# liruihui/Dis-PU

Hardware: AMD Instinct MI355X
Metric: upsampled points/sec (256->1024, 4x) (higher is better)
Workload: dtype f32; 1 GPU; BASELINE configs[1]: 32 patches x 256 points per GPU, generator forward 256->1024 (4x), fp32; patches_per_gpu=32, global_patches=32, weights=xavier-uniform seed 1234, zero bias, parallelism=patch-sharded x1

## Files before the change

### dis-pu_amd/_lib.py

```python
import ctypes as C
import os

_HERE = os.path.dirname(os.path.abspath(__file__))
LIB_PATH = os.path.join(_HERE, "lib", "libdispu_hip.so")

ABI_VERSION = 5
ARITH_PLAIN = 0
ARITH_CONTRACT = 1
ARITH_PINNED_EXP = 2
MESH_BRUTE_FORCE = 8
MESH_TILE = 64

_vp, _i, _sz, _l = C.c_void_p, C.c_int, C.c_size_t, C.c_long

SIGNATURES = {
    "dispu_version": (_i, []),
    "dispu_error_string": (C.c_char_p, [_i]),
    "dispu_event_record": (_i, [_vp, _vp]),
    "dispu_stream_wait_event": (_i, [_vp, _vp]),
    "dispu_memset_async": (_i, [_vp, _i, _sz, _vp]),
    "dispu_fps_scratch_bytes": (_sz, [_i, _i, _i]),
    "dispu_fps": (_i, [_i, _i, _i, _vp, _vp, _vp, _i, _vp]),
    "dispu_fps_ws": (_i, [_i, _i, _i, _vp, _vp, _sz, _vp, _i, _vp]),
    "dispu_fps_segments_scratch_bytes": (_sz, [_i, _vp, _vp]),
# ... 39 lines not shown
    "dispu_sa_fused": (_i, [_i, _i, _i, _i, _i, _vp, _vp, _vp, _vp, _i, _vp, _vp, _vp, _vp, _vp, _vp, _vp]),
    "dispu_edge_conv_fused": (_i, [_i, _i, _i, _i, _vp, _l, _vp, _i, _i, _vp, _vp, _vp, _vp, _vp, _i, _vp, _vp]),
    "dispu_group_center": (_i, [_l, _i, _i, _vp, _vp, _vp]),
    "dispu_pool_nsample": (_i, [_l, _i, _i, _i, _vp, _vp, _vp, _vp]),
    "dispu_idw_weights": (_i, [_l, _vp, _vp, _vp]),
    "dispu_l2_normalize_rows": (_i, [_l, _i, _vp, _vp, _vp]),
    "dispu_scale_add": (_i, [_l, _vp, C.c_float, _vp, _vp, _vp]),
    "dispu_edge_feature": (_i, [_l, _i, _i, _i, _vp, _l, _vp, _i, _i, _vp, _l, _vp]),
    "dispu_row_mean_max": (_i, [_i, _i, _vp, _vp, _vp, _vp]),
    "dispu_repulsion": (_i, [_l, _i, _i, _i, C.c_float, _vp, _vp, _vp, _vp]),
    "dispu_linear_small_k": (_i, [_l, _i, _i, _vp, _l, _vp, _vp, _i, _vp, _l, _vp]),
    "dispu_linear_small_n": (_i, [_l, _i, _i, _vp, _l, _vp, _vp, _i, _vp, _l, _vp, _l, _vp]),
    "dispu_edge_dense_conv": (_i, [_i, _i, _i, _vp, _l, _vp, _i, _i, _vp, _vp, _vp, _vp, _vp, _vp, _vp, _l, _vp]),
    "dispu_stem_block": (_i, [_i, _i, _i, _vp, _l, _i, _i, _vp, _vp, _vp, _vp, _vp, _vp, _vp, _l, _vp, _vp, _vp, _i, _vp, _l, _vp, _vp, _vp, _vp,
                              _l, _vp]),
    "dispu_edge_dense_conv_valu": (_i, [_i, _i, _i, _vp, _l, _vp, _i, _i, _vp, _vp, _vp, _vp, _vp, _vp, _vp, _l, _vp]),
    "dispu_dup_grid": (_i, [_i, _i, _i, _i, _vp, _l, _vp, _vp, _vp, _vp, _l, _vp]),
    "dispu_ps_prep": (_i, [_l, _i, _vp, _vp, _vp, _vp, _l, _vp, _l, _vp]),
    "dispu_ps_gather_sub_relu": (_i, [_l, _i, _i, _i, _vp, _vp, _l, _vp, _l, _vp, _l, _vp]),
    "dispu_ps_skip_max": (_i, [_l, _i, _i, _i, _vp, _vp, _vp, _l, _vp, _l, _vp]),
    "dispu_ps_weight_net": (_i, [_l, _i, _i, _i, _vp, _vp, _vp, _vp, _vp, _vp, _vp, _vp]),
    "dispu_ps_point_matmul": (_i, [_l, _i, _i, _i, _vp, _l, _vp, _vp, _l, _vp]),
    "dispu_ps_local": (_i, [_l, _i, _i, _i, _vp, _vp, _vp, _l, _vp, _vp, _vp, _vp, _vp, _vp, _vp, _vp, _vp]),
    "dispu_knn_patch": (_i, [_i, _i, _i, _i, _vp, _vp, _vp, _vp]),
    "dispu_normalize_patches": (_i, [_i, _i, _vp, _vp, _vp, _vp, _vp]),
    "dispu_denormalize_patches": (_i, [_i, _i, _vp, _vp, _vp, _vp, _vp]),
    "dispu_knn_patch_segments": (_i, [_i, _vp, _vp, _vp, _vp, _i, _vp, _vp, _vp, _vp]),
    "dispu_normalize_segments": (_i, [_i, _vp, _vp, _vp, _vp, _vp, _vp, _vp]),
    "dispu_attention": (_i, [_i, _i, _i, _i, _vp, _l, _vp, _l, _vp, _l, C.c_float, _vp, _l, _vp]),
    "dispu_attention_fwd_lse": (_i, [_i, _i, _i, _i, _vp, _l, _vp, _l, _vp, _l, C.c_float, _vp, _l, _vp, _vp]),
    "dispu_attention_bwd": (_i, [_i, _i, _i, _i, _vp, _l, _vp, _l, _vp, _l, C.c_float, _vp, _l, _vp, _vp, _l, _vp, _l, _vp, _l, _vp, _l,
                                 _vp, _vp]),
    "dispu_attention_project": (_i, [_i, _i, _i, _i, _vp, _l, _vp, _l, _vp, _l, C.c_float, _vp, _vp, _i, _vp, _l, _vp]),
    "dispu_softmax_rows": (_i, [_l, _i, C.c_float, _vp, _l, _vp]),
    "dispu_linear_tn_bf16_stream_scratch_floats": (_l, [_i, _i, _i]),
    "dispu_linear_tn_bf16_stream": (_i, [_i, _i, _i, _vp, _l, _vp, _l, _i, _vp, _l, _i, _vp, _vp, _l, _vp]),
    "dispu_bf16_pack": (_i, [_i, _i, _vp, _l, _i, _vp, _vp]),
    "dispu_linear_bf16_stream": (_i, [_i, _i, _i, _vp, _l, _i, _vp, _l, _vp, _i, _vp, _l, _i, _i, _l, _vp]),
    "dispu_linear_bf16": (_i, [_i, _i, _i, _i, _vp, _l, _l, _vp, _l, _l, _i, _vp, _i, _vp, _l, _l, _vp, _l, _l, _vp, _l, _l, _vp]),
    "dispu_linear_tn_bf16_scratch_floats": (_l, [_i, _i, _i, _i]),
    "dispu_linear_tn_bf16": (_i, [_i, _i, _i, _i, _vp, _l, _l, _vp, _l, _l, _vp, _l, _l, _i, _vp, _vp, _l, _vp]),
    "dispu_bf16x3_split_weights": (_i, [_i, _i, _vp, _l, _vp, _vp]),
    "dispu_linear_bf16x3": (_i, [_i, _i, _i, _vp, _l, _vp, _vp, _i, _vp, _l, _vp, _l, _vp, _l, _vp]),
    "dispu_debug_x3_kernel": (None, [_i]),
    "dispu_linear_tn_scratch_floats": (_l, [_i, _i, _i, _i]),
    "dispu_linear_tn": (_i, [_i, _i, _i, _i, _vp, _l, _l, _vp, _l, _l, _vp, _l, _l, _i, _vp, _vp, _l, _vp]),
    "dispu_ps_local_grad": (_i, [_l, _i] + [_vp] * 3 + [_l] + [_vp] * 14),
    "dispu_tn_defer": (_i, [_vp]),
    "dispu_tn_reduce_grouped": (_i, [_i, _vp, _vp, _vp]),
    "dispu_act_bias_grad_scratch_floats": (_l, [_l, _i]),
    "dispu_act_bias_grad": (_i, [_l, _i, _vp, _l, _vp, _l, _i, _vp, _l, _vp, _i, _vp, _l, _vp]),
    "dispu_max_k": (_i, [_l, _i, _i, _vp, _l, _vp, _l, _vp]),
    "dispu_max_k_grad": (_i, [_l, _i, _i, _vp, _l, _vp, _l, _vp, _l, _vp, _l, _i, _vp]),
    "dispu_max_k_grad_tail": (_i, [_l, _i, _i, _i, _vp, _l, _vp, _l, _vp, _l, _vp, _l, _vp]),
    "dispu_edge_feature_grad": (_i, [_l, _i, _i, _i, _vp, _l, _vp, _i, _i, _vp, _l, _vp]),
    "dispu_dup_sum_grad": (_i, [_i, _i, _i, _i, _vp, _l, _vp, _l, _vp]),
    "dispu_ps_group": (_i, [_l, _i, _i, _i, _vp, _vp, _vp, _l, _vp, _l, _vp]),
    "dispu_ps_group_grad": (_i, [_l, _i, _i, _i, _vp, _vp, _l, _vp, _vp, _l, _vp]),
    "dispu_ps_point_matmul_grad": (_i, [_l, _i, _i, _i, _vp, _l, _vp, _vp, _l, _vp, _l, _vp, _vp]),
    "dispu_softmax_rows_grad": (_i, [_l, _i, C.c_float, _vp, _l, _vp, _l, _vp]),
    "dispu_bn_scratch_bytes": (_l, [_l, _i]),
    "dispu_bn_train": (_i, [_l, _i, _vp, _l, _vp, _vp, C.c_float, C.c_float, _i, _vp, _l, _vp, _vp, _vp, _vp, _l, _vp]),
    "dispu_bn_train_grad": (_i, [_l, _i, _vp, _l, _vp, _l, _vp, _l, _vp, _vp, _i, _vp, _l, _vp, _vp, _vp, _vp, _l, _vp]),
    "dispu_sigmoid_offset": (_i, [_l, _vp, _vp, _vp, _vp]),
    "dispu_sigmoid_offset_grad": (_i, [_l, _vp, _vp, _vp, _vp, _vp]),
    "dispu_repulsion_grad": (_i, [_l, _i, _i, C.c_float, C.c_float, _vp, _vp, _vp, _vp]),
# ... 175 lines not shown
```

### dis-pu_amd/csrc/attention.hip

```cpp
#include "common.h"

namespace dispu {

typedef float f32x16 __attribute__((ext_vector_type(16)));

constexpr int FA_D = 64, FA_TK = 32, FA_LDK = FA_D + 1;
constexpr int FA_STAGE = FA_TK * FA_LDK + FA_TK * FA_D;

constexpr int FA_BPN = 256;
#ifdef FA_STAMPS
__device__ unsigned long long fa_stamps[16];
#endif

template <bool BP>
__global__ __launch_bounds__(512) void flash_attention_kernel(int m, int nk, const float* __restrict__ Q, long ldq,
                                                               const float* __restrict__ K, long ldk,
                                                               const float* __restrict__ V, long ldv, float scale,
                                                               float* __restrict__ O, long ldo,
                                                               const float* __restrict__ Wbp, const float* __restrict__ bbp) {
    extern __shared__ __attribute__((aligned(16))) float lds[];
    const int lane = threadIdx.x & 63, wave = threadIdx.x >> 6;
    int cloud = blockIdx.y, qblk = blockIdx.x;
    if ((gridDim.y & 7u) == 0) {
        const unsigned lin = blockIdx.x + gridDim.x * blockIdx.y, slot = lin >> 3;
        cloud = (int)((lin & 7u) * (gridDim.y >> 3) + slot / gridDim.x);
        qblk = (int)(slot % gridDim.x);
    }
    const float* __restrict__ kb = K + (size_t)cloud * nk * ldk;
    const float* __restrict__ vb = V + (size_t)cloud * nk * ldv;
    const int ntile = nk / FA_TK;

    if (wave >= 4) {
        const int tid = threadIdx.x - 256;
        float4 pk[2], pv[2];
        auto load_tile = [&](int k0) {
#pragma unroll
            for (int it = 0; it < 2; ++it) {
                const int e = tid + it * 256, key = e >> 4, c4 = e & 15;
                pk[it] = *reinterpret_cast<const float4*>(kb + (size_t)(k0 + key) * ldk + c4 * 4);
                pv[it] = *reinterpret_cast<const float4*>(vb + (size_t)(k0 + key) * ldv + c4 * 4);
            }
        };
        auto store_tile = [&](int stage) {
            float* Kt = lds + stage * FA_STAGE;
            float* Vt = Kt + FA_TK * FA_LDK;
#pragma unroll
            for (int it = 0; it < 2; ++it) {
                const int e = tid + it * 256, key = e >> 4, c4 = e & 15;
                Kt[key * FA_LDK + c4 * 4 + 0] = pk[it].x;
                Kt[key * FA_LDK + c4 * 4 + 1] = pk[it].y;
                Kt[key * FA_LDK + c4 * 4 + 2] = pk[it].z;
                Kt[key * FA_LDK + c4 * 4 + 3] = pk[it].w;
                *reinterpret_cast<float4*>(&Vt[key * FA_D + c4 * 4]) = pv[it];
            }
        };
        load_tile(0);
        if constexpr (BP) {
            float* Wl = lds + 2 * FA_STAGE;
#pragma unroll
            for (int h = 0; h < 4; ++h) {
                float4 w[4];
#pragma unroll
                for (int u = 0; u < 4; ++u) w[u] = *reinterpret_cast<const float4*>(Wbp + (size_t)(tid + (h * 4 + u) * 256) * 4);
#pragma unroll
                for (int u = 0; u < 4; ++u) *reinterpret_cast<float4*>(Wl + (size_t)(tid + (h * 4 + u) * 256) * 4) = w[u];
            }
        }
        store_tile(0);
        if (ntile > 1) load_tile(FA_TK);
        __syncthreads();
        for (int t = 0; t < ntile; ++t) {
            if (t + 1 < ntile) {
                store_tile((t + 1) & 1);
                if (t + 2 < ntile) load_tile((t + 2) * FA_TK);
            }
            __syncthreads();
        }
        return;
    }

    const int qrow = qblk * 128 + wave * 32 + (lane & 31);
    const int kh = lane >> 5, li = lane & 31;
    const bool qok = qrow < m;
    const float* __restrict__ qp = Q + ((size_t)cloud * m + (qok ? qrow : 0)) * ldq;

    const float scale2 = scale * 1.4426950408889634f;
    float qf[32];
#pragma unroll
    for (int s4 = 0; s4 < 16; ++s4) {
        const float4 v = *reinterpret_cast<const float4*>(qp + s4 * 4);
        qf[2 * s4] = (kh ? v.y : v.x) * scale2;
        qf[2 * s4 + 1] = (kh ? v.w : v.z) * scale2;
    }

    f32x16 oacc[2];
#pragma unroll
    for (int c = 0; c < 2; ++c)
#pragma unroll
        for (int r = 0; r < 16; ++r) oacc[c][r] = 0.f;
    float mrun = -__builtin_inff(), lsum = 0.f;

    __syncthreads();
#ifdef FA_STAMPS
    unsigned long long fa_s = 0, fa_sm = 0, fa_pv = 0, fa_bar = 0;
#define FA_T(v) __builtin_amdgcn_sched_barrier(0); const unsigned long long v = __builtin_readcyclecounter(); __builtin_amdgcn_sched_barrier(0)
#else
#define FA_T(v)
#endif
    for (int t = 0; t < ntile; ++t) {
        FA_T(c0);
        const float* Kt = lds + (t & 1) * FA_STAGE;
        const float* Vt = Kt + FA_TK * FA_LDK;
        f32x16 sacc;
#pragma unroll
        for (int r = 0; r < 16; ++r) sacc[r] = 0.f;
#pragma unroll
        for (int s = 0; s < 32; ++s) sacc = __builtin_amdgcn_mfma_f32_32x32x2f32(Kt[li * FA_LDK + 2 * s + kh], qf[s], sacc, 0, 0, 0);
        FA_T(c1);
        float mx = fmaxf(fmaxf(sacc[0], sacc[1]), sacc[2]);
#pragma unroll
        for (int r = 3; r < 15; r += 2) mx = fmaxf(fmaxf(mx, sacc[r]), sacc[r + 1]);
        mx = fmaxf(mx, sacc[15]);
        mx = fmaxf(mx, __shfl_xor(mx, 32, 64));
        const float mnew = fmaxf(mrun, mx);
        const float alpha = __builtin_amdgcn_exp2f(mrun - mnew);
        float rs = 0.f;
#pragma unroll
        for (int r = 0; r < 16; ++r) { sacc[r] = __builtin_amdgcn_exp2f(sacc[r] - mnew); rs += sacc[r]; }
        lsum = lsum * alpha + rs;
        mrun = mnew;
        if (__any(alpha != 1.0f)) {
#pragma unroll
            for (int c = 0; c < 2; ++c)
#pragma unroll
                for (int r = 0; r < 16; ++r) oacc[c][r] = oacc[c][r] * alpha;
        }
        FA_T(c2);
#pragma unroll
        for (int r = 0; r < 16; ++r) {
            const int key = (r & 3) + 8 * (r >> 2) + 4 * kh;
#pragma unroll
            for (int c = 0; c < 2; ++c)
                oacc[c] = __builtin_amdgcn_mfma_f32_32x32x2f32(Vt[key * FA_D + c * 32 + li], sacc[r], oacc[c], 0, 0, 0);
        }
        FA_T(c3);
        __syncthreads();
#ifdef FA_STAMPS
        { FA_T(c4); fa_s += c1 - c0; fa_sm += c2 - c1; fa_pv += c3 - c2; fa_bar += c4 - c3; }
#endif
    }
#ifdef FA_STAMPS
    if (blockIdx.x == 3 && blockIdx.y == 1 && lane == 0) {
        fa_stamps[wave * 4 + 0] = fa_s; fa_stamps[wave * 4 + 1] = fa_sm; fa_stamps[wave * 4 + 2] = fa_pv; fa_stamps[wave * 4 + 3] = fa_bar;
    }
#endif
    const float ltot = lsum + __shfl_xor(lsum, 32, 64);
    const float inv = 1.0f / ltot;
    float* __restrict__ op = O + ((size_t)cloud * m + (qok ? qrow : 0)) * ldo;
    if constexpr (!BP) {
        if (qok) {
#pragma unroll
            for (int c = 0; c < 2; ++c)
#pragma unroll
                for (int r = 0; r < 16; ++r) op[c * 32 + (r & 3) + 8 * (r >> 2) + 4 * kh] = oacc[c][r] * inv;
        }
    } else {
        const float* Wl = lds + 2 * FA_STAGE;
#pragma unroll
        for (int c = 0; c < 2; ++c)
#pragma unroll
            for (int r = 0; r < 16; ++r) oacc[c][r] = oacc[c][r] * inv;
#pragma unroll 1
        for (int ot = 0; ot < FA_BPN / 32; ot += 2) {
            f32x16 y0, y1;
#pragma unroll
            for (int r = 0; r < 16; ++r) { y0[r] = 0.f; y1[r] = 0.f; }
#pragma unroll
            for (int c = 0; c < 2; ++c)
#pragma unroll
                for (int r = 0; r < 16; ++r) {
                    const int d = c * 32 + (r & 3) + 8 * (r >> 2) + 4 * kh;
                    y0 = __builtin_amdgcn_mfma_f32_32x32x2f32(Wl[d * FA_BPN + ot * 32 + li], oacc[c][r], y0, 0, 0, 0);
                    y1 = __builtin_amdgcn_mfma_f32_32x32x2f32(Wl[d * FA_BPN + ot * 32 + 32 + li], oacc[c][r], y1, 0, 0, 0);
                }
            if (qok) {
#pragma unroll
                for (int g = 0; g < 4; ++g) {
                    const int o0 = ot * 32 + 8 * g + 4 * kh;
                    const float4 b0 = *reinterpret_cast<const float4*>(bbp + o0), b1 = *reinterpret_cast<const float4*>(bbp + o0 + 32);
                    float4 v0, v1;
                    v0.x = fmaxf(y0[4 * g + 0] + b0.x, 0.f); v0.y = fmaxf(y0[4 * g + 1] + b0.y, 0.f);
                    v0.z = fmaxf(y0[4 * g + 2] + b0.z, 0.f); v0.w = fmaxf(y0[4 * g + 3] + b0.w, 0.f);
                    v1.x = fmaxf(y1[4 * g + 0] + b1.x, 0.f); v1.y = fmaxf(y1[4 * g + 1] + b1.y, 0.f);
                    v1.z = fmaxf(y1[4 * g + 2] + b1.z, 0.f); v1.w = fmaxf(y1[4 * g + 3] + b1.w, 0.f);
                    *reinterpret_cast<float4*>(op + o0) = v0;
                    *reinterpret_cast<float4*>(op + o0 + 32) = v1;
                }
            }
        }
    }
}

}

using namespace dispu;

DISPU_EXPORT int dispu_attention(int b, int m, int nk, int d, const float* Q, long ldq, const float* K, long ldk, const float* V,
                                 long ldv, float scale, float* O, long ldo, void* stream) {
    if (b < 0 || m <= 0 || nk <= 0 || d != 64 || (nk % 32) != 0 || (ldq & 3) || (ldk & 3) || (ldv & 3) ||
        ((((uintptr_t)Q) | ((uintptr_t)K) | ((uintptr_t)V)) & 15))
        return (int)hipErrorInvalidValue;
    if (b == 0) return 0;
    hipLaunchKernelGGL((flash_attention_kernel<false>), dim3((m + 127) / 128, b), dim3(512), 2 * FA_STAGE * sizeof(float),
                       (hipStream_t)stream, m, nk, Q, ldq, K, ldk, V, ldv, scale, O, ldo, (const float*)nullptr, (const float*)nullptr);
    return (int)hipGetLastError();
}

DISPU_EXPORT int dispu_attention_project(int b, int m, int nk, int d, const float* Q, long ldq, const float* K, long ldk,
                                         const float* V, long ldv, float scale, const float* W, const float* bias, int n_out,
                                         float* Y, long ldy, void* stream) {
    if (b < 0 || m <= 0 || nk <= 0 || d != 64 || n_out != FA_BPN || (nk % 32) != 0 || (ldq & 3) || (ldk & 3) || (ldv & 3) ||
        (ldy & 3) || !W || !bias ||
        ((((uintptr_t)Q) | ((uintptr_t)K) | ((uintptr_t)V) | ((uintptr_t)W) | ((uintptr_t)bias) | ((uintptr_t)Y)) & 15))
        return (int)hipErrorInvalidValue;
    if (b == 0) return 0;
    constexpr size_t bytes = (size_t)(2 * FA_STAGE + FA_D * FA_BPN) * sizeof(float);
    static DevOnce attr;      
    if (attr.needed()) {
        DISPU_TRY(hipFuncSetAttribute(reinterpret_cast<const void*>(flash_attention_kernel<true>),
                                      hipFuncAttributeMaxDynamicSharedMemorySize, (int)bytes));
        attr.done();
    }
    hipLaunchKernelGGL((flash_attention_kernel<true>), dim3((m + 127) / 128, b), dim3(512), bytes, (hipStream_t)stream, m, nk, Q, ldq,
                       K, ldk, V, ldv, scale, Y, ldy, W, bias);
    return (int)hipGetLastError();
}
```

### dis-pu_amd/generator.py

```python
import contextlib
import math

import numpy as np
import torch

from . import _lib

K_NEIGH = 16
GROWTH = 24
DENSE_BLOCKS = 4
BN_EPS = 1e-3


def gen_grid(up_ratio):
    sq = int(math.sqrt(up_ratio)) + 1
    for i in range(sq, 0, -1):
        if up_ratio % i == 0:
            num_x, num_y = i, up_ratio // i
            break
    gx = np.linspace(-0.2, 0.2, num_x, dtype=np.float32)
    gy = np.linspace(-0.2, 0.2, num_y, dtype=np.float32)
    x, y = np.meshgrid(gx, gy)
    return np.stack([x, y], -1).reshape(-1, 2).astype(np.float32)


class _Opts(object):
    patch_num_point = 256
    up_ratio = 4


class Generator(object):

    MAX_POINTS = 2048 * 256

    def __init__(self, opts=None, is_training=False, name="Generator", params=None, device=None):
        self.opts = opts if opts is not None else _Opts()
        self.is_training = is_training
        self.name = name
        self.num_point = int(self.opts.patch_num_point)
        self.up_ratio = int(self.opts.up_ratio)
        if self.up_ratio != 4:
            raise NotImplementedError("the shipped generator graph is built for up_ratio 4 (DisPU/configs.py)")
        self.out_num_point = self.num_point * self.up_ratio
        self.device = torch.device(device if device is not None else "cuda:0")
        if self.device.type == "cuda" and self.device.index is None:
            self.device = torch.device("cuda", torch.cuda.current_device())
        self.P = {}
        self._ws = {}
        self.profile = None
        self.fused_local = True
        self.fused_attention = True
        self.fused_project = True
        self.split_bf16 = False
        self._planes = {}
        self.split_up3 = True
        self.branches = True
        self._aux = None
        self.fused_residual = True
        self.fused_heads = True
        self.keep_intermediates = False
        self.chain_inputs = True
        self.fused_stem = True
        self.return_views = False
        self.fine_out = None
        self._trainer = None
        if params is not None:
            self.load_params(params)

    def load_params(self, params):
        dev = self.device
        if self.is_training:
            from .train import Trainer, TrainOpts
            topts = TrainOpts()
            for k in dir(self.opts):
                if not k.startswith("_"):
                    setattr(topts, k, getattr(self.opts, k))
            self._trainer = Trainer(opts=topts, params=params, device=dev)
            self.P = self._trainer.P
            return
        self.P = {k: torch.from_numpy(np.ascontiguousarray(v, np.float32)).to(dev) for k, v in params.items()}
        self._planes = {}
        bn = "refine/PointShuffle/weight_net/wconv0/bn/"
        g, b = params[bn + "gamma"].astype(np.float64), params[bn + "beta"].astype(np.float64)
        mu, var = params[bn + "moving_mean"].astype(np.float64), params[bn + "moving_variance"].astype(np.float64)
        scale = g / np.sqrt(var + BN_EPS)
        self.bn_scale = torch.from_numpy(scale.astype(np.float32)).to(dev)
        self.bn_shift = torch.from_numpy((b - mu * scale).astype(np.float32)).to(dev)
        self.grid = torch.from_numpy(gen_grid(self.up_ratio)).to(dev)
        w1 = self.P["generator/upshuffle_0/conv1/weights"]
        self.w_up_feat = w1[:480].contiguous()
        self.w_up_grid = w1[480:482].contiguous()
        w0 = self.P["refine/PointShuffle/conv0/weights"]
        self.w_c0_feat = w0[6:134].contiguous()
        nlp = "refine/PointShuffle/PointShuffle/"
        self.w_up3 = torch.cat([self.P[nlp + "conv_kv/weights"], self.P[nlp + "conv_query/weights"], self.w_c0_feat], dim=1).contiguous()
        self.b_up3 = torch.cat([self.P[nlp + "conv_kv/biases"], self.P[nlp + "conv_query/biases"],
                                torch.zeros(128, dtype=torch.float32, device=dev)]).contiguous()
        wsk = self.P["refine/PointShuffle/skip/weights"]
        self.w_skip_pad = torch.cat([wsk, torch.zeros((10, wsk.shape[1]), dtype=torch.float32, device=dev)], dim=0).contiguous()

    def _w(self, scope):
        return self.P[scope + "/weights"], self.P[scope + "/biases"]

    def _workspace(self, B, N):
        key = (B, N)
        ws = self._ws.get(key)
        if ws is not None:
            return ws
        dev, f32, i32 = self.device, torch.float32, torch.int32
        M = N * self.up_ratio
        rn, rm, k = B * N, B * M, K_NEIGH

        def E(*shape, dtype=f32):
            return torch.empty(shape, dtype=dtype, device=dev)

        ws = dict(
            feat=E(rn, 480), prep=E(rn, 48), prep_b=E(rn, 48), kidx=E(rn, k + 1, dtype=i32), h256=E(rn, 256),
            up256=E(rm, 256), up128=E(rm, 128), c256=E(rm, 256), c64=E(rm, 64), coarse=E(B, M, 3),
            psidx=E(rm, k, dtype=i32), up3=E(rm, 320), att=E(rm, 64), nl=E(rm, 256),
            skipin=torch.zeros((rm, 144), dtype=f32, device=dev), skip=E(rm, 256), am=E(rm, 128),
            fp=E(rm, 2048), aft=E(rm, 256), agg=E(rm, 256),
            f256=E(rm, 256), f64=E(rm, 64), fine=E(B, M, 3))
        ws["kv"], ws["q"], ws["gm"] = ws["up3"][:, 0:128], ws["up3"][:, 128:192], ws["up3"][:, 192:320]
        self._ws[key] = ws
        return ws

    def _pair_buffers(self, B, N):
        key = ("pair", B, N)
        if key not in self._ws:
            rows = B * N * self.up_ratio * K_NEIGH
            E = lambda c: torch.empty((rows, c), dtype=torch.float32, device=self.device)
            self._ws[key] = (E(128), E(128), E(16))
        return self._ws[key]

    def _call(self, name, fn, *args):
        if self.profile is None:
            _lib.check(fn(*args), name)
            return
        e0, e1 = torch.cuda.Event(enable_timing=True), torch.cuda.Event(enable_timing=True)
        e0.record()
        _lib.check(fn(*args), name)
        e1.record()
        self.profile.append((name, e0, e1))

    def _linear(self, st, X, K, W, bias, act, Y, N, M=None, ldx=None, ldw=None, ldy=None, batch=1, sx=0, sw=0, sy=0,
                transb=0, R1=None, R2=None, xoff=0, woff=0, yoff=0):
        L = _lib.lib()
        M = X.shape[0] if M is None else M
        ldx = X.stride(0) if ldx is None else ldx
        ldw = W.stride(0) if ldw is None else ldw
        ldy = Y.stride(0) if ldy is None else ldy
        p = lambda t, off=0: _lib.C.c_void_p(t.data_ptr() + 4 * off) if t is not None else _lib.C.c_void_p(0)
        name = "linear"
        if self.profile is not None:
            t = L.dispu_linear_tile2(batch, M, K, N, int(bool(transb)))
            bm, bn = {128257: (128, 256), 128128: (128, 128), 64128: (64, 128), 128064: (128, 64)}.get(t, (64, 64))
# ... 121 lines not shown
            w3, b3_ = self._w(cs + "fc_layer1")
            w4, b4_ = self._w(cs + "fc_layer2")
            self._call("mlp_chain[coarse]", L.dispu_mlp_chain_dup, B, N, self.up_ratio, 256, 128, 256, 64, ptr(ws["h256"]), 256, ptr(self.w_up_grid),
                       ptr(b1), ptr(self.grid), ptr(w1), ptr(b1_), ptr(w2), ptr(b2_), ptr(w3), ptr(b3_), ptr(w4), ptr(b4_), ptr(ws["up128"]), 128,
                       0, None, 0, ptr(coarse), 3, st)
        elif heads:
            w1, b1_ = self._w("generator/upshuffle_0/conv2")
            w2, b2_ = self._w(cs + "fc_layer0")
            w3, b3_ = self._w(cs + "fc_layer1")
            w4, b4_ = self._w(cs + "fc_layer2")
            self._call("mlp_chain[coarse]", L.dispu_mlp_chain, rm, 256, 128, 256, 64, ptr(ws["up256"]), 256, ptr(w1), ptr(b1_), ptr(w2), ptr(b2_),
                       ptr(w3), ptr(b3_), ptr(w4), ptr(b4_), ptr(ws["up128"]), 128, 0, None, 0, ptr(coarse), 3, st)
        else:
            w, b = self._w("generator/upshuffle_0/conv2")
            self._linear(st, ws["up256"], 256, w, b, 1, ws["up128"], 128)
            w, b = self._w(cs + "fc_layer0")
            self._linear(st, ws["up128"], 128, w, b, 1, ws["c256"], 256)
            w, b = self._w(cs + "fc_layer1")
            self._linear(st, ws["c256"], 256, w, b, 1, ws["c64"], 64)
            w, b = self._w(cs + "fc_layer2")
            self._call("coarse", L.dispu_linear_small_n, rm, 64, 3, ptr(ws["c64"]), 64, ptr(w), ptr(b), 0, None, 0, ptr(coarse), 3, st)

        ps = "refine/PointShuffle/"
        up128 = ws["up128"]
        br = self.branches
        if br:
            if self._aux is None:
                self._aux = (torch.cuda.Stream(device=self.device), torch.cuda.Event(), torch.cuda.Event(), torch.cuda.Event())
            aux, ev_fork, ev_up3, ev_nl = self._aux
            ev_fork.record(torch.cuda.current_stream(self.device))
            aux.wait_event(ev_fork)
        with (torch.cuda.stream(aux) if br else contextlib.nullcontext()):
            sb = _lib.C.c_void_p(aux.cuda_stream) if br else st
            if self.split_up3:
                self._linear(sb, up128, 128, self.w_up3, self.b_up3, 0, ws["up3"], 256)
                self._linear(sb, up128, 128, self.w_up3, self.b_up3[256:], 0, ws["up3"], 64, woff=256, yoff=256)
            else:
                self._linear(sb, up128, 128, self.w_up3, self.b_up3, 0, ws["up3"], 320)
            if br:
                ev_up3.record(aux)
            w_bp, b_bp = self._w(ps + "PointShuffle/conv_back_project")
            projected = False
            if self.fused_attention and M % 32 == 0 and self.fused_project:
                self._call("attention_project", L.dispu_attention_project, B, M, M, 64, ptr(ws["q"]), 320, ptr(ws["kv"]), 320,
                           off(ws["kv"], 64), 320, 0.125, ptr(w_bp), ptr(b_bp), 256, ptr(ws["nl"]), 256, sb)
                projected = True
            elif self.fused_attention and M % 32 == 0:
                self._call("attention", L.dispu_attention, B, M, M, 64, ptr(ws["q"]), 320, ptr(ws["kv"]), 320, off(ws["kv"], 64), 320,
                           0.125, ptr(ws["att"]), 64, sb)
            else:
                key = ("scores", B, N)
                if key not in self._ws:
                    self._ws[key] = torch.empty((B, M, M), dtype=torch.float32, device=self.device)
                s = self._ws[key]
                self._linear(sb, ws["q"], 64, ws["kv"], None, 0, s, M, M=M, ldx=320, ldw=320, ldy=M, batch=B, sx=M * 320,
                             sw=M * 320, sy=M * M, transb=1)
                self._call("softmax", L.dispu_softmax_rows, rm, M, 0.125, ptr(s), M, sb)
                self._linear(sb, s, M, ws["kv"], None, 0, ws["att"], 64, M=M, ldx=M, ldw=320, ldy=64, batch=B, sx=M * M,
                             sw=M * 320, sy=M * 64, woff=64)
            if not projected:
                self._linear(sb, ws["att"], 64, w_bp, b_bp, 1, ws["nl"], 256)
            if br:
                ev_nl.record(aux)
        nb = L.dispu_knn_xyz_scratch_bytes(B, M, M, k)
        if nb and ws.get("knn_scratch") is None:
            ws["knn_scratch"] = torch.empty((nb,), dtype=torch.uint8, device=self.device)
        self._call("knn_xyz", L.dispu_knn_xyz_ws, B, M, M, k, ptr(coarse), ptr(coarse), ptr(ws["psidx"]), None,
                   ptr(ws["knn_scratch"]) if nb else None, nb, _lib.ARITH_PLAIN, st)
        self._call("skip_max", L.dispu_ps_skip_max, rm, M, k, 128, ptr(ws["psidx"]), ptr(coarse), ptr(up128), 128, ptr(ws["skipin"]), 144, st)
        _, b = self._w(ps + "skip")
        self._linear(st, ws["skipin"], 144, self.w_skip_pad, b, 1, ws["skip"], 256)
        if br:
            torch.cuda.current_stream(self.device).wait_event(ev_up3)
        w0, b0 = self._w(ps + "conv0")
        self._call("ps_prep", L.dispu_ps_prep, rm, 128, ptr(coarse), ptr(w0), ptr(b0), ptr(ws["gm"]), 320, ptr(ws["am"]), 128, st)
        w1, b1 = self._w(ps + "conv1")
        ww, bw = self._w(ps + "weight_net/wconv0")
        if self.fused_local:
            self._call("ps_local", L.dispu_ps_local, rm, M, k, 128, ptr(ws["psidx"]), ptr(coarse), ptr(ws["gm"]), 320, ptr(ws["am"]),
# ... 61 lines not shown
```

### include/dispu_hip.h

```cpp
#ifndef DISPU_HIP_H
#define DISPU_HIP_H

#include <stddef.h>

#ifdef __cplusplus
extern "C" {
#endif

#define DISPU_ARITH_PLAIN 0
#define DISPU_ARITH_CONTRACT 1
#define DISPU_ARITH_PINNED_EXP 2
#define DISPU_KNN_LANE_PER_QUERY 4
#define DISPU_MESH_BRUTE_FORCE 8
#define DISPU_MESH_TILE 64

int dispu_version(void);
int dispu_event_record(void* event, void* stream);
int dispu_stream_wait_event(void* stream, void* event);
int dispu_memset_async(void* dst, int value, size_t bytes, void* stream);
const char* dispu_error_string(int code);


size_t dispu_fps_scratch_bytes(int b, int n, int m);
int dispu_fps(int b, int n, int m, const float* inp, float* temp, int* out, int arith, void* stream);
// ... 90 lines not shown
                         float* Y, long ldy, void* stream);
int dispu_linear_small_n(long rows, int K, int N, const float* X, long ldx, const float* W, const float* bias, int mode,
                         const float* R, long ldr, float* Y, long ldy, void* stream);
int dispu_edge_dense_conv(int npoints, int n_per_cloud, int C, const float* F, long ldf, const int* idx, int ldi, int ioff,
                          const float* W0, const float* b0, const float* W1, const float* b1, const float* W2,
                          const float* b2, float* Y, long ldy, void* stream);
int dispu_stem_block(int npoints, int n_per_cloud, int C, const float* F, long ldf, int ksel, int ioff, const float* W0, const float* b0,
                     const float* W1, const float* b1, const float* W2, const float* b2, float* Y, long ldy, int* idx_out, const float* Wp,
                     const float* bp, int k_old, float* P, long ldp, const float* xyz, const float* Wl, const float* bl, float* Lout,
                     long ldl, void* stream);
int dispu_edge_dense_conv_valu(int npoints, int n_per_cloud, int C, const float* F, long ldf, const int* idx, int ldi,
                               int ioff, const float* W0, const float* b0, const float* W1, const float* b1,
                               const float* W2, const float* b2, float* Y, long ldy, void* stream);
int dispu_dup_grid(int nclouds, int n, int co, int up, const float* H, long ldh, const float* Wg, const float* bias,
                   const float* grid, float* Y, long ldy, void* stream);
int dispu_ps_prep(long rows, int co, const float* xyz, const float* W0, const float* bias, float* G, long ldg, float* A,
                  long lda, void* stream);
int dispu_ps_gather_sub_relu(long rows, int n_per_cloud, int k, int c, const int* idx, const float* G, long ldg,
                             const float* A, long lda, float* X1, long ldx1, void* stream);
int dispu_ps_skip_max(long rows, int n_per_cloud, int k, int cf, const int* idx, const float* xyz, const float* feat,
                      long ldf, float* out, long ldo, void* stream);
int dispu_ps_weight_net(long rows, int n_per_cloud, int k, int t_n, const int* idx, const float* xyz, const float* Ww,
                        const float* bw, const float* scale, const float* shift, float* wv, void* stream);
int dispu_ps_point_matmul(long rows, int k, int c, int t_n, const float* X2, long ldx2, const float* wv, float* out,
                          long ldo, void* stream);
int dispu_ps_local(long npoints, int n_per_cloud, int k, int c, const int* idx, const float* xyz, const float* G, long ldg,
                   const float* A, const float* W1, const float* b1, const float* Ww, const float* bw, const float* scale,
                   const float* shift, float* out, void* stream);
int dispu_attention(int b, int m, int nk, int d, const float* Q, long ldq, const float* K, long ldk, const float* V,
                    long ldv, float scale, float* O, long ldo, void* stream);
int dispu_attention_project(int b, int m, int nk, int d, const float* Q, long ldq, const float* K, long ldk, const float* V,
                            long ldv, float scale, const float* W, const float* bias, int n_out, float* Y, long ldy,
                            void* stream);
int dispu_attention_fwd_lse(int b, int m, int nk, int d, const float* Q, long ldq, const float* K, long ldk, const float* V,
                            long ldv, float scale, float* O, long ldo, float* lse2, void* stream);
int dispu_attention_bwd(int b, int m, int nk, int d, const float* Q, long ldq, const float* K, long ldk, const float* V, long ldv,
                        float scale, const float* O, long ldo, const float* lse2, const float* dO, long lddo, float* dQ, long lddq,
                        float* dK, long lddk, float* dV, long lddv, float* dvec, void* stream);
int dispu_softmax_rows(long rows, int n, float mul, float* S, long lds, void* stream);

int dispu_mlp_chain(long rows, int K0, int N1, int N2, int N3, const float* X, long ldx, const float* W1, const float* b1,
                    const float* W2, const float* b2, const float* W3, const float* b3, const float* W4, const float* b4,
                    float* Y1, long ldy1, int mode, const float* R, long ldr, float* out, long ldo, void* stream);
int dispu_mlp_chain_sum3(long rows, int K0, int N1, int N2, int N3, const float* X, const float* X2, const float* X3, long ldx,
                         const float* W1, const float* b1, const float* W2, const float* b2, const float* W3, const float* b3,
                         const float* W4, const float* b4, float* Y1, long ldy1, int mode, const float* R, long ldr, float* out, long ldo,
                         void* stream);
int dispu_mlp_chain_dup(int nclouds, int n, int up, int K0, int N1, int N2, int N3, const float* H, long ldh, const float* Wg,
                        const float* bg, const float* grid, const float* W1, const float* b1, const float* W2, const float* b2,
                        const float* W3, const float* b3, const float* W4, const float* b4, float* Y1, long ldy1, int mode, const float* R,
                        long ldr, float* out, long ldo, void* stream);

int dispu_group_center(long rows, int ns, int c, float* grouped, const float* center, void* stream);
int dispu_sa_fused(int b, int n, int m, int ns, int c, const float* xyz, const float* new_xyz, const float* points, const int* idx,
                   int nl, const float* const* W, const float* const* bias, const float* const* scale, const float* const* shift,
                   const int* cout, float* out, void* stream);
int dispu_edge_conv_fused(int b, int n, int k, int c, const float* feat, long ldf, const int* idx, int ldi, int nl,
                          const float* const* W, const float* const* bias, const float* const* scale, const float* const* shift,
                          const int* cout, int act_last, float* out, void* stream);
int dispu_pool_nsample(long rows, int ns, int c, int mode, const float* X, const float* gxyz, float* out, void* stream);
int dispu_l2_normalize_rows(long rows, int c, const float* X, float* out, void* stream);
int dispu_scale_add(long n, const float* x, float alpha, const float* y, float* out, void* stream);
int dispu_idw_weights(long rows, const float* dist, float* weight, void* stream);
int dispu_edge_feature(long rows, int n_per_cloud, int k, int c, const float* F, long ldf, const int* idx, int ldi, int ioff,
                       float* out, long ldo, void* stream);
int dispu_row_mean_max(int b, int n, const float* x, float* mean, float* mx, void* stream);
// ... 191 lines not shown
```

Before: 36.10 million points/s.

## Fuse query projection into flash attention kernel and stream back-projection weights

Adds an attention variant that computes the query projection (128->64) inside the flash-attention kernel with MFMA from the raw features, so the separate query linear and its global-memory round trip are no longer needed. Producer waves now stage the back-projection weights into LDS in slices interleaved with the K/V tile pipeline, and the query weights temporarily occupy that same LDS region. The up3 weight layout is reordered so the query columns come last and can be skipped. The cost is extra per-block MFMA work and register pressure in the consumer waves, plus extra synchronisation around the shared LDS region.

After: 35.93 million points/s. No clear change (-0.5%).

```diff
diff --git a/dis-pu_amd/_lib.py b/dis-pu_amd/_lib.py
--- a/dis-pu_amd/_lib.py
+++ b/dis-pu_amd/_lib.py
@@ -95,6 +95,7 @@
     "dispu_attention_bwd": (_i, [_i, _i, _i, _i, _vp, _l, _vp, _l, _vp, _l, C.c_float, _vp, _l, _vp, _vp, _l, _vp, _l, _vp, _l, _vp, _l,
                                  _vp, _vp]),
     "dispu_attention_project": (_i, [_i, _i, _i, _i, _vp, _l, _vp, _l, _vp, _l, C.c_float, _vp, _vp, _i, _vp, _l, _vp]),
+    "dispu_attention_project_q": (_i, [_i, _i, _i, _i, _vp, _l, _vp, _vp, _vp, _l, _vp, _l, C.c_float, _vp, _vp, _i, _vp, _l, _vp]),
     "dispu_softmax_rows": (_i, [_l, _i, C.c_float, _vp, _l, _vp]),
     "dispu_linear_tn_bf16_stream_scratch_floats": (_l, [_i, _i, _i]),
     "dispu_linear_tn_bf16_stream": (_i, [_i, _i, _i, _vp, _l, _vp, _l, _i, _vp, _l, _i, _vp, _vp, _l, _vp]),
diff --git a/dis-pu_amd/csrc/attention.hip b/dis-pu_amd/csrc/attention.hip
--- a/dis-pu_amd/csrc/attention.hip
+++ b/dis-pu_amd/csrc/attention.hip
@@ -3,21 +3,26 @@
 namespace dispu {
 
 typedef float f32x16 __attribute__((ext_vector_type(16)));
+typedef float f32x4 __attribute__((ext_vector_type(4)));
 
 constexpr int FA_D = 64, FA_TK = 32, FA_LDK = FA_D + 1;
 constexpr int FA_STAGE = FA_TK * FA_LDK + FA_TK * FA_D;
 
 constexpr int FA_BPN = 256;
+constexpr int FA_WSL = 4;
+constexpr int FA_QK = 128;
 #ifdef FA_STAMPS
 __device__ unsigned long long fa_stamps[16];
 #endif
 
-template <bool BP>
+template <bool BP, bool PQ>
 __global__ __launch_bounds__(512) void flash_attention_kernel(int m, int nk, const float* __restrict__ Q, long ldq,
+                                                               const float* __restrict__ Wq, const float* __restrict__ bq,
                                                                const float* __restrict__ K, long ldk,
                                                                const float* __restrict__ V, long ldv, float scale,
                                                                float* __restrict__ O, long ldo,
                                                                const float* __restrict__ Wbp, const float* __restrict__ bbp) {
+    static_assert(BP || !PQ, "the query projection borrows the LDS region of W");
     extern __shared__ __attribute__((aligned(16))) float lds[];
     const int lane = threadIdx.x & 63, wave = threadIdx.x >> 6;
     int cloud = blockIdx.y, qblk = blockIdx.x;
@@ -32,13 +37,13 @@
 
     if (wave >= 4) {
         const int tid = threadIdx.x - 256;
-        float4 pk[2], pv[2];
+        f32x4 pk[2], pv[2];
         auto load_tile = [&](int k0) {
 #pragma unroll
             for (int it = 0; it < 2; ++it) {
                 const int e = tid + it * 256, key = e >> 4, c4 = e & 15;
-                pk[it] = *reinterpret_cast<const float4*>(kb + (size_t)(k0 + key) * ldk + c4 * 4);
-                pv[it] = *reinterpret_cast<const float4*>(vb + (size_t)(k0 + key) * ldv + c4 * 4);
+                pk[it] = *reinterpret_cast<const f32x4*>(kb + (size_t)(k0 + key) * ldk + c4 * 4);
+                pv[it] = *reinterpret_cast<const f32x4*>(vb + (size_t)(k0 + key) * ldv + c4 * 4);
             }
         };
         auto store_tile = [&](int stage) {
@@ -51,20 +56,26 @@
                 Kt[key * FA_LDK + c4 * 4 + 1] = pk[it].y;
                 Kt[key * FA_LDK + c4 * 4 + 2] = pk[it].z;
                 Kt[key * FA_LDK + c4 * 4 + 3] = pk[it].w;
-                *reinterpret_cast<float4*>(&Vt[key * FA_D + c4 * 4]) = pv[it];
-            }
+                *reinterpret_cast<f32x4*>(&Vt[key * FA_D + c4 * 4]) = pv[it];
+            }
+        };
+        f32x4 wsl[16 / FA_WSL];
+        float* Wl = lds + 2 * FA_STAGE;
+        auto load_w = [&](int sl) {
+#pragma unroll
+            for (int u = 0; u < 16 / FA_WSL; ++u) wsl[u] = *reinterpret_cast<const f32x4*>(Wbp + (size_t)(tid + (sl * (16 / FA_WSL) + u) * 256) * 4);
+        };
+        auto store_w = [&](int sl) {
+#pragma unroll
+            for (int u = 0; u < 16 / FA_WSL; ++u) *reinterpret_cast<f32x4*>(Wl + (size_t)(tid + (sl * (16 / FA_WSL) + u) * 256) * 4) = wsl[u];
         };
         load_tile(0);
-        if constexpr (BP) {
-            float* Wl = lds + 2 * FA_STAGE;
-#pragma unroll
-            for (int h = 0; h < 4; ++h) {
-                float4 w[4];
-#pragma unroll
-                for (int u = 0; u < 4; ++u) w[u] = *reinterpret_cast<const float4*>(Wbp + (size_t)(tid + (h * 4 + u) * 256) * 4);
-#pragma unroll
-                for (int u = 0; u < 4; ++u) *reinterpret_cast<float4*>(Wl + (size_t)(tid + (h * 4 + u) * 256) * 4) = w[u];
-            }
+        if constexpr (PQ) {
+            f32x4 w[8];
+#pragma unroll
+            for (int u = 0; u < 8; ++u) w[u] = *reinterpret_cast<const f32x4*>(Wq + (size_t)(tid + u * 256) * 4);
+#pragma unroll
+            for (int u = 0; u < 8; ++u) *reinterpret_cast<f32x4*>(Wl + (size_t)(tid + u * 256) * 4) = w[u];
         }
         store_tile(0);
         if (ntile > 1) load_tile(FA_TK);
@@ -74,7 +85,20 @@
                 store_tile((t + 1) & 1);
                 if (t + 2 < ntile) load_tile((t + 2) * FA_TK);
             }
+            if constexpr (BP) {
+                if (t >= 1 && t <= FA_WSL) store_w(t - 1);
+                if (t < FA_WSL) load_w(t);
+            }
             __syncthreads();
+        }
+        if constexpr (BP) {
+            if (ntile <= FA_WSL) {
+                for (int sl = ntile - 1; sl < FA_WSL; ++sl) {
+                    if (sl >= ntile) load_w(sl);
+                    store_w(sl);
+                }
+                __syncthreads();
+            }
         }
         return;
     }
@@ -86,11 +110,38 @@
 
     const float scale2 = scale * 1.4426950408889634f;
     float qf[32];
-#pragma unroll
-    for (int s4 = 0; s4 < 16; ++s4) {
-        const float4 v = *reinterpret_cast<const float4*>(qp + s4 * 4);
-        qf[2 * s4] = (kh ? v.y : v.x) * scale2;
-        qf[2 * s4 + 1] = (kh ? v.w : v.z) * scale2;
+    if constexpr (!PQ) {
+#pragma unroll
+        for (int s4 = 0; s4 < 16; ++s4) {
+            const float4 v = *reinterpret_cast<const float4*>(qp + s4 * 4);
+            qf[2 * s4] = (kh ? v.y : v.x) * scale2;
+            qf[2 * s4 + 1] = (kh ? v.w : v.z) * scale2;
+        }
+    } else {
+        float xf[FA_QK / 2];
+#pragma unroll
+        for (int s4 = 0; s4 < FA_QK / 4; ++s4) {
+            const float4 v = *reinterpret_cast<const float4*>(qp + s4 * 4);
+            xf[2 * s4] = kh ? v.y : v.x;
+            xf[2 * s4 + 1] = kh ? v.w : v.z;
+        }
+        __syncthreads();
+        const float* Wl = lds + 2 * FA_STAGE + 2 * ((li & 3) + 4 * (li >> 3)) + ((li >> 2) & 1);
+        f32x16 qa[2];
+#pragma unroll
+        for (int c = 0; c < 2; ++c)
+#pragma unroll
+            for (int r = 0; r < 16; ++r) qa[c][r] = 0.f;
+#pragma unroll
+        for (int t = 0; t < FA_QK / 2; ++t)
+#pragma unroll
+            for (int c = 0; c < 2; ++c) qa[c] = __builtin_amdgcn_mfma_f32_32x32x2f32(Wl[(2 * t + kh) * FA_D + c * 32], xf[t], qa[c], 0, 0, 0);
+#pragma unroll
+        for (int s4 = 0; s4 < 16; ++s4) {
+            const float4 v = *reinterpret_cast<const float4*>(bq + s4 * 4);
+            qf[2 * s4] = (qa[s4 >> 3][(2 * s4) & 15] + (kh ? v.y : v.x)) * scale2;
+            qf[2 * s4 + 1] = (qa[s4 >> 3][(2 * s4 + 1) & 15] + (kh ? v.w : v.z)) * scale2;
+        }
     }
 
     f32x16 oacc[2];
@@ -100,7 +151,7 @@
         for (int r = 0; r < 16; ++r) oacc[c][r] = 0.f;
     float mrun = -__builtin_inff(), lsum = 0.f;
 
-    __syncthreads();
+    if constexpr (!PQ) __syncthreads();
 #ifdef FA_STAMPS
     unsigned long long fa_s = 0, fa_sm = 0, fa_pv = 0, fa_bar = 0;
 #define FA_T(v) __builtin_amdgcn_sched_barrier(0); const unsigned long long v = __builtin_readcyclecounter(); __builtin_amdgcn_sched_barrier(0)
@@ -165,6 +216,7 @@
                 for (int r = 0; r < 16; ++r) op[c * 32 + (r & 3) + 8 * (r >> 2) + 4 * kh] = oacc[c][r] * inv;
         }
     } else {
+        if (ntile <= FA_WSL) __syncthreads();
         const float* Wl = lds + 2 * FA_STAGE;
 #pragma unroll
         for (int c = 0; c < 2; ++c)
@@ -211,8 +263,9 @@
         ((((uintptr_t)Q) | ((uintptr_t)K) | ((uintptr_t)V)) & 15))
         return (int)hipErrorInvalidValue;
     if (b == 0) return 0;
-    hipLaunchKernelGGL((flash_attention_kernel<false>), dim3((m + 127) / 128, b), dim3(512), 2 * FA_STAGE * sizeof(float),
-                       (hipStream_t)stream, m, nk, Q, ldq, K, ldk, V, ldv, scale, O, ldo, (const float*)nullptr, (const float*)nullptr);
+    hipLaunchKernelGGL((flash_attention_kernel<false, false>), dim3((m + 127) / 128, b), dim3(512), 2 * FA_STAGE * sizeof(float),
+                       (hipStream_t)stream, m, nk, Q, ldq, (const float*)nullptr, (const float*)nullptr, K, ldk, V, ldv, scale, O, ldo,
+                       (const float*)nullptr, (const float*)nullptr);
     return (int)hipGetLastError();
 }
 
@@ -227,11 +280,32 @@
     constexpr size_t bytes = (size_t)(2 * FA_STAGE + FA_D * FA_BPN) * sizeof(float);
     static DevOnce attr;      
     if (attr.needed()) {
-        DISPU_TRY(hipFuncSetAttribute(reinterpret_cast<const void*>(flash_attention_kernel<true>),
+        DISPU_TRY(hipFuncSetAttribute(reinterpret_cast<const void*>(flash_attention_kernel<true, false>),
                                       hipFuncAttributeMaxDynamicSharedMemorySize, (int)bytes));
         attr.done();
     }
-    hipLaunchKernelGGL((flash_attention_kernel<true>), dim3((m + 127) / 128, b), dim3(512), bytes, (hipStream_t)stream, m, nk, Q, ldq,
-                       K, ldk, V, ldv, scale, Y, ldy, W, bias);
+    hipLaunchKernelGGL((flash_attention_kernel<true, false>), dim3((m + 127) / 128, b), dim3(512), bytes, (hipStream_t)stream, m, nk, Q, ldq,
+                       (const float*)nullptr, (const float*)nullptr, K, ldk, V, ldv, scale, Y, ldy, W, bias);
     return (int)hipGetLastError();
 }
+
+DISPU_EXPORT int dispu_attention_project_q(int b, int m, int nk, int d, const float* X, long ldx, const float* Wq, const float* bq,
+                                           const float* K, long ldk, const float* V, long ldv, float scale, const float* W,
+                                           const float* bias, int n_out, float* Y, long ldy, void* stream) {
+    if (b < 0 || m <= 0 || nk <= 0 || d != 64 || n_out != FA_BPN || (nk % 32) != 0 || (ldx & 3) || (ldk & 3) || (ldv & 3) ||
+        (ldy & 3) || !W || !bias || !Wq || !bq ||
+        ((((uintptr_t)X) | ((uintptr_t)Wq) | ((uintptr_t)bq) | ((uintptr_t)K) | ((uintptr_t)V) | ((uintptr_t)W) | ((uintptr_t)bias) |
+          ((uintptr_t)Y)) & 15))
+        return (int)hipErrorInvalidValue;
+    if (b == 0) return 0;
+    constexpr size_t bytes = (size_t)(2 * FA_STAGE + FA_D * FA_BPN) * sizeof(float);
+    static DevOnce attr;
+    if (attr.needed()) {
+        DISPU_TRY(hipFuncSetAttribute(reinterpret_cast<const void*>(flash_attention_kernel<true, true>),
+                                      hipFuncAttributeMaxDynamicSharedMemorySize, (int)bytes));
+        attr.done();
+    }
+    hipLaunchKernelGGL((flash_attention_kernel<true, true>), dim3((m + 127) / 128, b), dim3(512), bytes, (hipStream_t)stream, m, nk, X, ldx,
+                       Wq, bq, K, ldk, V, ldv, scale, Y, ldy, W, bias);
+    return (int)hipGetLastError();
+}
diff --git a/dis-pu_amd/generator.py b/dis-pu_amd/generator.py
--- a/dis-pu_amd/generator.py
+++ b/dis-pu_amd/generator.py
@@ -53,7 +53,7 @@
         self.fused_project = True
         self.split_bf16 = False
         self._planes = {}
-        self.split_up3 = True
+        self.fused_query = True
         self.branches = True
         self._aux = None
         self.fused_residual = True
@@ -93,9 +93,9 @@
         w0 = self.P["refine/PointShuffle/conv0/weights"]
         self.w_c0_feat = w0[6:134].contiguous()
         nlp = "refine/PointShuffle/PointShuffle/"
-        self.w_up3 = torch.cat([self.P[nlp + "conv_kv/weights"], self.P[nlp + "conv_query/weights"], self.w_c0_feat], dim=1).contiguous()
-        self.b_up3 = torch.cat([self.P[nlp + "conv_kv/biases"], self.P[nlp + "conv_query/biases"],
-                                torch.zeros(128, dtype=torch.float32, device=dev)]).contiguous()
+        self.w_up3 = torch.cat([self.P[nlp + "conv_kv/weights"], self.w_c0_feat, self.P[nlp + "conv_query/weights"]], dim=1).contiguous()
+        self.b_up3 = torch.cat([self.P[nlp + "conv_kv/biases"], torch.zeros(128, dtype=torch.float32, device=dev),
+                                self.P[nlp + "conv_query/biases"]]).contiguous()
         wsk = self.P["refine/PointShuffle/skip/weights"]
         self.w_skip_pad = torch.cat([wsk, torch.zeros((10, wsk.shape[1]), dtype=torch.float32, device=dev)], dim=0).contiguous()
 
@@ -121,7 +121,7 @@
             skipin=torch.zeros((rm, 144), dtype=f32, device=dev), skip=E(rm, 256), am=E(rm, 128),
             fp=E(rm, 2048), aft=E(rm, 256), agg=E(rm, 256),
             f256=E(rm, 256), f64=E(rm, 64), fine=E(B, M, 3))
-        ws["kv"], ws["q"], ws["gm"] = ws["up3"][:, 0:128], ws["up3"][:, 128:192], ws["up3"][:, 192:320]
+        ws["kv"], ws["gm"], ws["q"] = ws["up3"][:, 0:128], ws["up3"][:, 128:256], ws["up3"][:, 256:320]
         self._ws[key] = ws
         return ws
 
@@ -309,19 +309,21 @@
             aux.wait_event(ev_fork)
         with (torch.cuda.stream(aux) if br else contextlib.nullcontext()):
             sb = _lib.C.c_void_p(aux.cuda_stream) if br else st
-            if self.split_up3:
-                self._linear(sb, up128, 128, self.w_up3, self.b_up3, 0, ws["up3"], 256)
-                self._linear(sb, up128, 128, self.w_up3, self.b_up3[256:], 0, ws["up3"], 64, woff=256, yoff=256)
-            else:
-                self._linear(sb, up128, 128, self.w_up3, self.b_up3, 0, ws["up3"], 320)
+            self._linear(sb, up128, 128, self.w_up3, self.b_up3, 0, ws["up3"], 256)
             if br:
                 ev_up3.record(aux)
             w_bp, b_bp = self._w(ps + "PointShuffle/conv_back_project")
-            projected = False
-            if self.fused_attention and M % 32 == 0 and self.fused_project:
+            projected = self.fused_attention and M % 32 == 0 and self.fused_project
+            if not (projected and self.fused_query):
+                self._linear(sb, up128, 128, self.w_up3, self.b_up3[256:], 0, ws["up3"], 64, woff=256, yoff=256)
+            if projected and self.fused_query:
+                w_q, b_q = self._w(ps + "PointShuffle/conv_query")
+                self._call("attention_project", L.dispu_attention_project_q, B, M, M, 64, ptr(up128), 128, ptr(w_q), ptr(b_q),
+                           ptr(ws["kv"]), 320, off(ws["kv"], 64), 320, 0.125, ptr(w_bp), ptr(b_bp), 256,
+                           ptr(ws["nl"]), 256, sb)
+            elif projected:
                 self._call("attention_project", L.dispu_attention_project, B, M, M, 64, ptr(ws["q"]), 320, ptr(ws["kv"]), 320,
                            off(ws["kv"], 64), 320, 0.125, ptr(w_bp), ptr(b_bp), 256, ptr(ws["nl"]), 256, sb)
-                projected = True
             elif self.fused_attention and M % 32 == 0:
                 self._call("attention", L.dispu_attention, B, M, M, 64, ptr(ws["q"]), 320, ptr(ws["kv"]), 320, off(ws["kv"], 64), 320,
                            0.125, ptr(ws["att"]), 64, sb)
diff --git a/include/dispu_hip.h b/include/dispu_hip.h
--- a/include/dispu_hip.h
+++ b/include/dispu_hip.h
@@ -146,6 +146,9 @@
 int dispu_attention_project(int b, int m, int nk, int d, const float* Q, long ldq, const float* K, long ldk, const float* V,
                             long ldv, float scale, const float* W, const float* bias, int n_out, float* Y, long ldy,
                             void* stream);
+int dispu_attention_project_q(int b, int m, int nk, int d, const float* X, long ldx, const float* Wq, const float* bq,
+                              const float* K, long ldk, const float* V, long ldv, float scale, const float* W, const float* bias,
+                              int n_out, float* Y, long ldy, void* stream);
 int dispu_attention_fwd_lse(int b, int m, int nk, int d, const float* Q, long ldq, const float* K, long ldk, const float* V,
                             long ldv, float scale, float* O, long ldo, float* lse2, void* stream);
 int dispu_attention_bwd(int b, int m, int nk, int d, const float* Q, long ldq, const float* K, long ldk, const float* V, long ldv,
```
